# gyhandy/Neural-Sim-NeRF

Hardware: AMD Instinct MI355X
Metric: Mray-samples/sec at 400x400, 64+128 samples, 8x256 MLP (higher is better)
Workload: dtype f16x2

## Files before the change

### neural_sim_nerf_amd/csrc/nsr_kernels.hip

```cpp
#include <hip/hip_runtime.h>
#include <stdint.h>
#include "nsr_device.h"

#if !defined(NSR_UNIT_F32) && !defined(NSR_UNIT_H2) && !defined(NSR_UNIT_B3) && !defined(NSR_UNIT_X16)
#define NSR_UNIT_F32 1
#define NSR_UNIT_H2 1
#define NSR_UNIT_B3 1
#define NSR_UNIT_X16 1
#endif
#ifndef NSR_UNIT_F32
#define NSR_UNIT_F32 0
#endif
#ifndef NSR_UNIT_H2
#define NSR_UNIT_H2 0
#endif
#ifndef NSR_UNIT_B3
#define NSR_UNIT_B3 0
#endif
#ifndef NSR_UNIT_X16
#define NSR_UNIT_X16 0
#endif
#define NSR_CAT_(a, b) a##b
#define NSR_CAT(a, b) NSR_CAT_(a, b)

// ... 87 lines not shown
  const char* p = rg.smem + rg.cslot * kSlabBytes + lane * 16;
#pragma unroll
  for (int c = 0; c < 4; ++c) A0[c] = *(const f32x4*)(p + c * 1024);
}

template <int U>
__device__ __forceinline__ void ring_load_quarter(const Ring& rg, f32x4 (&A)[4], int lane) {
  const char* p = rg.smem + rg.cslot * kSlabBytes + U * kStepBytes + lane * 16;
#pragma unroll
  for (int c = 0; c < 4; ++c) A[c] = *(const f32x4*)(p + c * 1024);
}

template <int NS = kRingSlots>
__device__ __forceinline__ void ring_advance(Ring& rg, f32x4 (&A)[4], int lane) {
  asm volatile("s_waitcnt vmcnt(%0) lgkmcnt(0)" ::"n"(4 * (NS - 2)) : "memory");
#ifndef NSR_EXP_NOBARRIER
  __builtin_amdgcn_s_barrier();
#endif
  rg.cslot = (rg.cslot + 1 == NS) ? 0 : rg.cslot + 1;
  const char* p = rg.smem + rg.cslot * kSlabBytes + lane * 16;
#pragma unroll
  for (int c = 0; c < 4; ++c) A[c] = *(const f32x4*)(p + c * 1024);
}

#define NSR_MFMA(a, b, c) __builtin_amdgcn_mfma_f32_32x32x2f32((a), (b), (c), 0, 0, 0)
__device__ __forceinline__ f32x16 mfma_op(float a, float b, f32x16 c) { return __builtin_amdgcn_mfma_f32_32x32x2f32(a, b, c, 0, 0, 0); }
__device__ __forceinline__ f32x4 mfma_op(float a, float b, f32x4 c) { return __builtin_amdgcn_mfma_f32_16x16x4f32(a, b, c, 0, 0, 0); }

template <int NMO, int KK0, int KK1, bool ZERO = false, int NACC, typename BOp, typename AccT>
__device__ __forceinline__ void consume(const f32x4 (&A)[4], int step, BOp bop, AccT (&acc)[NACC]) {
#pragma unroll
  for (int kk = KK0; kk < KK1; ++kk)
#pragma unroll
    for (int c = 0; c < 4; ++c) {
      const int n = 4 * step + c, tq = n / NMO, mo = n % NMO;
      if (ZERO && tq == 0 && kk == 0) acc[mo] = mfma_op(A[c][kk], bop(4 * tq + kk), AccT{0});
      else acc[mo] = mfma_op(A[c][kk], bop(4 * tq + kk), acc[mo]);
    }
}

#define NSR_PIN() __builtin_amdgcn_sched_barrier(0)
#define NSR_SGB(mask, n) __builtin_amdgcn_sched_group_barrier((mask), (n), 0)
#define NSR_MASK_VALU 0x002
#define NSR_MASK_SALU 0x004
#define NSR_MASK_MFMA 0x008
#define NSR_MASK_VMEM 0x010
#define NSR_MASK_DSRD 0x100
template <int N_MFMA>
__device__ __forceinline__ void step_pattern() {
#pragma unroll
  for (int i = 0; i < N_MFMA; ++i) {
    NSR_SGB(NSR_MASK_MFMA, 1);
    NSR_SGB(NSR_MASK_DSRD, 1);
    NSR_SGB(NSR_MASK_VALU, 2);
  }
}
template <int N_MFMA>
__device__ __forceinline__ void step_pattern_dma() {
#pragma unroll
  for (int i = 0; i < N_MFMA; ++i) {
    NSR_SGB(NSR_MASK_MFMA, 1);
    NSR_SGB(NSR_MASK_DSRD, 1);
    NSR_SGB(NSR_MASK_VMEM, 1);
    NSR_SGB(NSR_MASK_SALU, 3);
    NSR_SGB(NSR_MASK_VALU, 2);
  }
}

template <int NMO, int NTQ, int NS = kRingSlots, bool ZERO = false, int NACC, typename BOp, typename AccT>
__device__ __forceinline__ void seg(Ring& rg, f32x4 (&A0)[4], f32x4 (&A1)[4], BOp bop, AccT (&acc)[NACC],
                                    int lane) {
  static_assert((NMO * NTQ) % 16 == 0, "a segment is a whole number of slabs");
#pragma unroll
  for (int s = 0; s < NMO * NTQ / 4; s += 4) {
    NSR_PIN(); ring_load_quarter<1>(rg, A1, lane); consume<NMO, 0, 4, ZERO>(A0, s, bop, acc);     step_pattern<16>();
    NSR_PIN(); ring_load_quarter<2>(rg, A0, lane); consume<NMO, 0, 4, ZERO>(A1, s + 1, bop, acc); step_pattern<16>();
    NSR_PIN(); ring_load_quarter<3>(rg, A1, lane); consume<NMO, 0, 4, ZERO>(A0, s + 2, bop, acc); step_pattern<16>();
    NSR_PIN(); consume<NMO, 0, 1, ZERO>(A1, s + 3, bop, acc);
    NSR_PIN(); ring_advance<NS>(rg, A0, lane);
    ring_issue<NS>(rg); consume<NMO, 1, 4, ZERO>(A1, s + 3, bop, acc); step_pattern_dma<12>();
    NSR_PIN();
  }
}

template <int NG>
struct BRegs16 {
  const f32x16 (&v)[NG];
  __device__ __forceinline__ float operator()(int t) const { return v[t >> 4][t & 15]; }
};
template <int N>
struct BArr {
  const float (&v)[N];
  __device__ __forceinline__ float operator()(int t) const { return v[t]; }
};
struct BViews {
  const f32x16 (&v)[8];
  const float (&ed)[16];
  __device__ __forceinline__ float operator()(int t) const { return t < 128 ? v[(t & 127) >> 4][t & 15] : ed[t & 15]; }
};

__device__ __forceinline__ int aux_half(int lane) { return opaque_v((lane >> 5) * 4); }

template <int NMO>
__device__ __forceinline__ void load_bias(const float* bias, int h4 , f32x16 (&acc)[NMO]) {
#pragma unroll
  for (int mo = 0; mo < NMO; ++mo)
#pragma unroll
    for (int rq = 0; rq < 4; ++rq) {
      f32x4 v = *(const f32x4*)(bias + (mo * 4 + rq) * 8 + h4);
      acc[mo][rq * 4 + 0] = v[0];
      acc[mo][rq * 4 + 1] = v[1];
      acc[mo][rq * 4 + 2] = v[2];
      acc[mo][rq * 4 + 3] = v[3];
    }
}

#include "nsr_b3.inc"
#include "nsr_h2.inc"

constexpr int kMlpF32 = 0;
constexpr int kMlpB3 = 1;
constexpr int kMlpH2 = 2;

template <int NMO>
__device__ __forceinline__ uint4 relu_mask(const f32x16 (&acc)[NMO]) {
  unsigned w[4] = {0u, 0u, 0u, 0u};
#pragma unroll
  for (int mo = 0; mo < NMO; ++mo)
#pragma unroll
    for (int r = 0; r < 16; ++r) {
      const int on = max(__float_as_int(acc[mo][r]), 0) - 1;
      w[mo >> 1] = __builtin_amdgcn_alignbit(w[mo >> 1], (unsigned)on, 31);
    }
  return make_uint4(w[0], w[1], w[2], w[3]);
}

__device__ __forceinline__ float enc_trig(float a, int k) {
  const double kMagic = 6755399441055744.0;
  const double t = (double)a * 0.63661977236758134308;
  const double tm = t + kMagic;
  const int n = __double2loint(tm) + k;
  const double f = t - (tm - kMagic);
  const float r = (float)(f * 1.57079632679489661923);
  const float z = r * r;
  float ps = __builtin_fmaf(-1.9515295891e-4f, z, 8.3321608736e-3f);
  ps = __builtin_fmaf(ps, z, -1.6666654611e-1f);
  ps = __builtin_fmaf(ps * z, r, r);
  float pc = __builtin_fmaf(2.443315711809948e-5f, z, -1.388731625493765e-3f);
  pc = __builtin_fmaf(pc, z, 4.166664568298827e-2f);
  pc = __builtin_fmaf(pc * z, z, __builtin_fmaf(-0.5f, z, 1.0f));
  const float v = (n & 1) ? pc : ps;
  return __uint_as_float(__float_as_uint(v) ^ ((unsigned)(n & 2) << 30));
}

__device__ __forceinline__ float enc_domain(float x, int nfreq) {
  return __builtin_fabsf(x) < ldexpf(1.0f, 25 - nfreq) ? x : __builtin_nanf("");
}

__device__ __forceinline__ float enc_poison(float px, float py, float pz, float vx, float vy, float vz) {
  const float a = (enc_domain(px, kMultires) * 0.0f + enc_domain(py, kMultires) * 0.0f) + enc_domain(pz, kMultires) * 0.0f;
  const float b = (enc_domain(vx, kMultiresViews) * 0.0f + enc_domain(vy, kMultiresViews) * 0.0f) +
                  enc_domain(vz, kMultiresViews) * 0.0f;
  return __builtin_fabsf(a + b);
}

template <bool CAPTURE, int MODE = kMlpF32>
__device__ __forceinline__ void mlp_pass(Ring& rg, const float* aux, f32x4 (&A0)[4], f32x4 (&A1)[4], int lane,
                                         float px, float py, float pz, float vx, float vy, float vz,
                                         float (&raw)[4], uint4* mask_dst = nullptr , int mask_tid = 0,
                                         long long* tp = nullptr ) {
#ifdef NSR_PHASE_TIMING
  long long tpl = clock64();
#define NSR_TP(i) do { if (tp) { const long long t_ = clock64(); tp[i] += t_ - tpl; tpl = t_; } } while (0)
#else
#define NSR_TP(i) do { } while (0)
#endif
  const int h = lane >> 5;
  const int h4 = aux_half(lane);
  const float poison = enc_poison(px, py, pz, vx, vy, vz);
  float e[32];
  float ed[16];
  {
    const float p[3] = {px, py, pz};
    const float v[3] = {vx, vy, vz};
#pragma unroll
    for (int L = 0; L < kMultires; ++L)
#pragma unroll
      for (int ax = 0; ax < 3; ++ax) e[3 * L + ax] = enc_trig(enc_domain(p[ax], kMultires) * (float)(1 << L), h);
#pragma unroll
    for (int L = 0; L < kMultiresViews; ++L)
#pragma unroll
      for (int ax = 0; ax < 3; ++ax) ed[3 * L + ax] = enc_trig(enc_domain(v[ax], kMultiresViews) * (float)(1 << L), h);
    e[30] = h ? pz : px;
    e[31] = h ? 0.0f : py;
    ed[12] = h ? vz : vx;
    ed[13] = h ? 0.0f : vy;
    ed[14] = 0.0f;
    ed[15] = 0.0f;
  }

  f32x16 acc[8];
  f32x16 in[8];
  auto enc_src = [&](int kb, int i) { return e[(8 * kb + i) & 31]; };
  auto in_src = [&](int kb, int i) { return in[(kb >> 1) & 7][8 * (kb & 1) + i]; };
  constexpr bool B3 = MODE == kMlpB3;
  constexpr bool H2M = MODE == kMlpH2;
  float amax = 0.0f;
  const float* h2s = aux + kAuxH2Scale;
#if NSR_H2_SCHED == 3 && !defined(NSR_EXP_H2_NOFRAG) && !defined(NSR_EXP_H2_HALFBARRIER) && !defined(NSR_EXP_H2_NOSPLIT)
  constexpr bool TAIL = H2M && !CAPTURE;
#else
  constexpr bool TAIL = false;
#endif
  static_assert(kAuxBiasV == kAuxBias + 9 * 256, "the views layer's bias follows feature_linear's: 'bias of layer L + 1' for L = 8");
  NSR_TP(0);
  load_bias<8>(aux + kAuxBias, h4, acc);
  NSR_TP(2);
  if constexpr (B3) gemm_b3<8, 2>(rg, A0, A1, enc_src, acc, lane);
  else if constexpr (TAIL)
    gemm_h2_tail<4>(rg, A0, A1, enc_src, H2Scale{{h2s[0], 0.0f}, 4}, acc, lane, amax, H2Tail{acc, in, 0, h2_lds_base(aux + kAuxBias + 256, h4)});
  else if constexpr (H2M) gemm_h2<8, 4>(rg, A0, A1, enc_src, H2Scale{{h2s[0], 0.0f}, 4}, acc, lane, amax);
  else seg<8, 8>(rg, A0, A1, BArr<32>{e}, acc, lane);
  NSR_TP(1);
  if (CAPTURE) mask_dst[mask_tid] = relu_mask<8>(acc);
  if constexpr (!TAIL) {
#pragma unroll
    for (int mo = 0; mo < 8; ++mo) in[mo] = relu16(acc[mo]);
  }

  float alpha_part = 0.0f;
#pragma unroll 1
  for (int L = 1; L <= 8; ++L) {
    if constexpr (!TAIL) load_bias<8>(aux + kAuxBias + L * 256, h4, acc);
    NSR_TP(2);
    if (L == 5) {
      if constexpr (B3) gemm_b3<8, 2>(rg, A0, A1, enc_src, acc, lane);
      else if constexpr (H2M) gemm_h2<8, 4>(rg, A0, A1, enc_src, H2Scale{{h2s[9], 0.0f}, 4}, acc, lane, amax);
      else seg<8, 8>(rg, A0, A1, BArr<32>{e}, acc, lane);
      NSR_TP(1);
    }
    if (L == 8) {
      const float* wa = aux + kAuxWAlpha;
#pragma unroll
      for (int tq = 0; tq < 32; ++tq) {
        f32x4 w = *(const f32x4*)(wa + tq * 8 + h4);
#pragma unroll
        for (int kk = 0; kk < 4; ++kk)
          alpha_part = __builtin_fmaf(w[kk], in[(4 * tq + kk) >> 4][(4 * tq + kk) & 15], alpha_part);
      }
    }
    if constexpr (B3) gemm_b3<8, 8>(rg, A0, A1, in_src, acc, lane);
    else if constexpr (TAIL)
      gemm_h2_tail<16>(rg, A0, A1, in_src, H2Scale{{h2s[L], 0.0f}, 16}, acc, lane, amax,
                       H2Tail{acc, in, (L == 8) ? (int)0x80000000 : 0, h2_lds_base(aux + kAuxBias + (L + 1) * 256, h4)});
    else if constexpr (H2M) gemm_h2<8, 16>(rg, A0, A1, in_src, H2Scale{{h2s[L], 0.0f}, 16}, acc, lane, amax);
    else seg<8, 32>(rg, A0, A1, BRegs16<8>{in}, acc, lane);
    NSR_TP(1);
    if (CAPTURE && L < 8) mask_dst[L * 256 + mask_tid] = relu_mask<8>(acc);
    if constexpr (!TAIL) {
      const int thr = (L == 8) ? (int)0x80000000 : 0;
#pragma unroll
      for (int mo = 0; mo < 8; ++mo) in[mo] = clamp_bits16(acc[mo], thr);
    }
  }

  f32x16 av[4];
  if constexpr (TAIL) {
#pragma unroll
    for (int mo = 0; mo < 4; ++mo) av[mo] = acc[mo];
  } else {
    load_bias<4>(aux + kAuxBiasV, h4, av);
  }
  NSR_TP(2);
  if constexpr (B3) {
    auto v_src = [&](int kb, int i) {
      return kb < 16 ? in[(kb >> 1) & 7][8 * (kb & 1) + i] : (kb < 18 ? ed[(8 * (kb - 16) + i) & 15] : 0.0f);
    };
    gemm_b3<4, 5>(rg, A0, A1, v_src, av, lane);
  } else if constexpr (H2M) {
    auto v_src = [&](int kb, int i) { return kb < 16 ? in[(kb >> 1) & 7][8 * (kb & 1) + i] : ed[(8 * (kb - 16) + i) & 15]; };
    gemm_h2<4, 18>(rg, A0, A1, v_src, H2Scale{{h2s[10], h2s[11]}, 16}, av, lane, amax);
  } else {
    seg<4, 36>(rg, A0, A1, BViews{in, ed}, av, lane);
  }
  NSR_TP(1);
  if (CAPTURE) mask_dst[8 * 256 + mask_tid] = relu_mask<4>(av);

  float part[4] = {0.0f, 0.0f, 0.0f, alpha_part};
  if constexpr (H2M) {
    const float ov = amax > kH2Max ? __builtin_nanf("") : 0.0f;
    part[0] = part[1] = part[2] = ov;
    part[3] = alpha_part + ov;
  }
#pragma unroll
  for (int c = 0; c < 3; ++c) {
    const float* wr = aux + kAuxWRgb + c * 128;
#pragma unroll
    for (int mo = 0; mo < 4; ++mo)
#pragma unroll
      for (int rq = 0; rq < 4; ++rq) {
        f32x4 w = *(const f32x4*)(wr + (mo * 4 + rq) * 8 + h4);
#pragma unroll
        for (int ri = 0; ri < 4; ++ri)
          part[c] = __builtin_fmaf(w[ri], fmaxf(av[mo][rq * 4 + ri], 0.0f), part[c]);
      }
  }
#pragma unroll
  for (int c = 0; c < 4; ++c) {
    float other = __shfl_xor(part[c], 32);
    float lo_half = h ? other : part[c];
    float hi_half = h ? part[c] : other;
    raw[c] = ((lo_half + hi_half) + aux[(c < 3) ? (kAuxBRgb + c) : kAuxBAlpha]) + poison;
  }
  NSR_TP(3);
#undef NSR_TP
}

template <int NSS, int NFS>
struct ItemStateT {
  static constexpr int kNS = NSS, kNF = NFS;
  float tcoarse[NSS];
  float ufine[128];
  float ray[2][16];
  float zc[2][NSS];
  float rawc[2][NSS][4];
  float w0[2][NSS];
  float cdf[2][NSS];
  float zs[2][128];
  float zf[2][NFS];
  float rawf[2][NFS][4];
  float alpha[2][NFS];
  float wf[2][NFS];
  float tf[2][NFS];
  float om[2][NFS];
  float bwd_scratch[2][NFS][2];
  float psum[2][NFS / 32][12];
  float gnorm[2];
  float res[2][8];
};
typedef ItemStateT<64, 192> ItemState;
typedef ItemStateT<128, 256> ItemStateBig;
static_assert(sizeof(ItemState) == 23048, "the YCB-V layout is part of the shipped kernels' LDS budget");
template <int NS> struct ItemStateFor { typedef ItemState type; };
template <> struct ItemStateFor<128> { typedef ItemStateBig type; };

__device__ __forceinline__ float sigmoidf_(float x) { return 1.0f / (1.0f + expf(-x)); }

template <int S, int R = 2, int STRIDE = S, typename ST>
__device__ __forceinline__ void composite(ST& st, const float* z, float* raw, float* wout, float* tout, int tid,
                                          const float* noise = nullptr ,
                                          long long row0 = 0, int valid = R) {
  static_assert(S % 8 == 0, "scan is unrolled by 8");
  for (int idx = tid; idx < R * S; idx += 256) {
    const int r = idx / S, i = idx - r * S;
    const float* zr = z + r * STRIDE;
    float dist = (i < S - 1) ? (zr[i + 1] - zr[i]) : 1e10f;
    dist = dist * st.ray[r][11];
    float* q = raw + (r * STRIDE + i) * 4;
    if (noise) q[3] = q[3] + noise[(row0 + (r < valid ? r : 0)) * S + i];
    const float sigma = fmaxf(q[3], 0.0f);
    const float a = 1.0f - expf(-sigma * dist);
    st.alpha[r][i] = a;
    st.om[r][i] = (1.0f - a) + 1e-10f;
    q[0] = sigmoidf_(q[0]);
    q[1] = sigmoidf_(q[1]);
    q[2] = sigmoidf_(q[2]);
  }
  __syncthreads();
  if ((tid & 63) == 0 && tid < 64 * R) {
    const int r = tid >> 6;
    double T = 1.0;
#pragma unroll 1
    for (int i0 = 0; i0 < S; i0 += 8) {
      double f[8];
#pragma unroll
      for (int k = 0; k < 8; ++k) f[k] = (double)st.om[r][i0 + k];
#pragma unroll
      for (int k = 0; k < 8; ++k) {
        tout[r * STRIDE + i0 + k] = (float)T;
        T = T * f[k];
      }
    }
  }
  __syncthreads();
  if (tid < 64 * R) {
    const int r = tid >> 6, l = tid & 63;
    const float* zr = z + r * STRIDE;
    const float* q = raw + r * STRIDE * 4;
    float cr = 0.f, cg = 0.f, cb = 0.f, depth = 0.f, acc = 0.f;
#pragma unroll
    for (int i = l; i < S; i += 64) {
      const float w = st.alpha[r][i] * tout[r * STRIDE + i];
      wout[r * STRIDE + i] = w;
      cr = cr + w * q[i * 4 + 0];
      cg = cg + w * q[i * 4 + 1];
      cb = cb + w * q[i * 4 + 2];
      depth = depth + w * zr[i];
      acc = acc + w;
    }
#pragma unroll
    for (int m = 32; m >= 1; m >>= 1) {
      cr += __shfl_xor(cr, m); cg += __shfl_xor(cg, m); cb += __shfl_xor(cb, m);
      depth += __shfl_xor(depth, m); acc += __shfl_xor(acc, m);
    }
    if (l == 0) {
      const float qd = depth / acc;
      float disp;
      if (qd != qd) disp = qd;
      else disp = 1.0f / fmaxf(1e-10f, qd);
      if (st.ray[r][12] != 0.0f) {
        const float bg = 1.0f - acc;
        cr = cr + bg; cg = cg + bg; cb = cb + bg;
      }
      st.res[r][0] = cr; st.res[r][1] = cg; st.res[r][2] = cb;
      st.res[r][3] = disp; st.res[r][4] = acc; st.res[r][5] = depth;
    }
  }
  __syncthreads();
}

template <int R, int NI, int NS, typename ST, typename BinsFn>
__device__ __forceinline__ void sample_pdf_item_ns(ST& st, const float* ufine, const float* w, int wstride, BinsFn bins,
                                                   int64_t* inds_out, int64_t inds_stride, int tid, int valid_rays,
                                                   const float* u_rays, long long row0, int write_mask) {
// ... 251 lines not shown
    __syncthreads();
    if (tid < 2 * NS) st.zc[r][i] = zn;
    __syncthreads();
  }
}

__device__ __forceinline__ void gen_ray(const float* __restrict__ c2w, float fx, float fy, float cx, float cy,
                                        int row, int col, float (&o)[3], float (&d)[3]) {
  const float dx = ((float)col - cx) / fx;
  const float dy = -(((float)row - cy) / fy);
  const float dz = -1.0f;
#pragma unroll
  for (int a = 0; a < 3; ++a) {
    d[a] = ((dx * c2w[a * 4 + 0]) + (dy * c2w[a * 4 + 1])) + (dz * c2w[a * 4 + 2]);
    o[a] = c2w[a * 4 + 3];
  }
}

struct RenderArgs {
  const float* nets;
  long long net_stride;
  const float* aux[2];
  const float* tcoarse;
  const float* ufine;
  const float* rays_o;
  const float* rays_d;
  const float* c2w;
  float fx, fy, cx, cy;
  int H, W;
  long long n_rays;
  float near_, far_;
  int fine;
  int camera;
  int white_bkgd;
  int lindisp;
  float *rgb, *disp, *acc, *rgb0, *disp0, *acc0, *z_std;
  float *dbg_w0, *dbg_zs, *dbg_zf, *dbg_raw0, *dbg_raw;
  long long* dbg_inds;
  float* zf_scratch;
  int chunk;
  unsigned* sched_flags;
  unsigned* status;
  int super_lg;
  int spin_max;
  unsigned epoch;
  unsigned* epoch_counter;
  unsigned long long* work_counter;
  const float* viewdirs;
  const float* t_rand;
  const float* u_rays;
  const float* noise0;
  const float* noise1;
  const float* near_rays;
  const float* far_rays;
  unsigned long long* ovf_items;
  unsigned* ovf_stat;
  unsigned ovf_cap;
  const unsigned long long* item_list;
  const unsigned* item_count;
  unsigned item_cap;
};

__device__ __forceinline__ void load_aux(char* smem, const RenderArgs& a, int tid) {
  float* dst = (float*)(smem + kLdsAux);
  for (int i = tid; i < kAuxFloats; i += 256) {
    dst[i] = a.aux[0][i];
    dst[kAuxFloats + i] = a.aux[1][i];
  }
}

#if NSR_UNIT_F32
__global__ void k_set_args(const RenderArgs a, RenderArgs* dst) {
  *dst = a;
  *a.work_counter = 0ull;
  if (a.ovf_stat) a.ovf_stat[0] = 0u;
  if (a.epoch_counter) dst->epoch = *a.epoch_counter = *a.epoch_counter % 4094u + 1u;
}
#endif

constexpr long long kItemMask = (1ll << 62) - 1;
__device__ __forceinline__ long long queue_next_item(const RenderArgs& q) {
  const unsigned long long v = atomicAdd(q.work_counter, 1ull);
  if (q.item_list) {
    unsigned n = *q.item_count;
    n = n < q.item_cap ? n : q.item_cap;
    return v < (unsigned long long)n ? (long long)q.item_list[v] : -1ll;
  }
  return v < (unsigned long long)((q.n_rays + 1) >> 1) ? (long long)(v | (3ull << 62)) : -1ll;
}
__device__ __forceinline__ long long queue_item_of(const RenderArgs& q, unsigned long long v) {
  if (q.item_list) {
    unsigned n = *q.item_count;
    n = n < q.item_cap ? n : q.item_cap;
    return v < (unsigned long long)n ? (long long)q.item_list[v] : -1ll;
  }
  return v < (unsigned long long)((q.n_rays + 1) >> 1) ? (long long)(v | (3ull << 62)) : -1ll;
}
__device__ __forceinline__ long long queue_items(const RenderArgs& q) {
  if (q.item_list) { const unsigned n = *q.item_count; return (long long)(n < q.item_cap ? n : q.item_cap); }
  return (q.n_rays + 1) >> 1;
}
__device__ __forceinline__ void range_mark(int* ovf, float chk, int lane) {
#ifndef NSR_EXP_NO_RANGE
  if (chk != chk && lane < 32) atomicAdd(ovf, 1);
#endif
}
__device__ __forceinline__ unsigned range_report(const RenderArgs& a, int* ovf, long long item, int valid) {
#ifdef NSR_EXP_NO_RANGE
  return 0u;
#endif
  const int p0 = ovf[0], p1 = valid == 2 ? ovf[1] : 0;
  if ((p0 | p1) != 0 && a.ovf_stat) {
    const unsigned long long mask = (p0 ? 1ull : 0ull) | (p1 ? 2ull : 0ull);
    const unsigned n = atomicAdd(a.ovf_stat, 1u);
    atomicAdd(a.ovf_stat + 1, (unsigned)(p0 + p1));
    if (n < a.ovf_cap) {
      a.ovf_items[n] = (unsigned long long)item | (mask << 62);
      atomicAdd(a.ovf_stat + 2, (unsigned)((p0 != 0) + (p1 != 0)));
    } else {
      atomicAdd(a.ovf_stat + 3, 1u);
      return (unsigned)mask;
    }
  }
  return 0u;
}
__device__ __forceinline__ void range_poison(const RenderArgs& a, long long ray0, unsigned mask) {
  const float qn = __builtin_nanf("");
  for (int r = 0; r < 2; ++r) {
    if (!((mask >> r) & 1u)) continue;
    const long long rr = ray0 + r;
    float* const v3[2] = {a.rgb, a.rgb0};
    float* const v1[5] = {a.disp, a.acc, a.disp0, a.acc0, a.z_std};
    for (int k = 0; k < 2; ++k) if (v3[k]) { v3[k][rr * 3] = qn; v3[k][rr * 3 + 1] = qn; v3[k][rr * 3 + 2] = qn; }
    for (int k = 0; k < 5; ++k) if (v1[k]) v1[k][rr] = qn;
  }
}

__device__ __forceinline__ void wave_lds_sync() {
  __builtin_amdgcn_fence(__ATOMIC_RELEASE, "wavefront");
  __builtin_amdgcn_wave_barrier();
  __builtin_amdgcn_fence(__ATOMIC_ACQUIRE, "wavefront");
}
__device__ __forceinline__ void lds_barrier() { asm volatile("s_waitcnt lgkmcnt(0)\n\ts_barrier" ::: "memory"); }

template <typename ST>
struct FwdItemExtra {
  float om[2][ST::kNS];
  float tf[2][ST::kNS];
  float zf[2][ST::kNF];
  float ray[2][16];
  float res[2][8];
  long long pend;
  long long next;
};

template <int S>
__device__ __forceinline__ void composite_wave(const float* ry, const float* zr, float* q, float* wr, float* tr, float* omr,
                                               int lane, const float* noise ,
                                               float (&res)[6]) {
  static_assert(S % 8 == 0, "scan is unrolled by 8");
  constexpr int K = (S + 63) / 64;
  float al[K];
#pragma unroll
  for (int k = 0; k < K; ++k) {
    const int i = lane + 64 * k;
    al[k] = 0.0f;
    if (i < S) {
      float dist = (i < S - 1) ? (zr[i + 1] - zr[i]) : 1e10f;
      dist = dist * ry[11];
      if (noise) q[i * 4 + 3] = q[i * 4 + 3] + noise[i];
      const float sigma = fmaxf(q[i * 4 + 3], 0.0f);
      const float a = 1.0f - expf(-sigma * dist);
      al[k] = a;
      omr[i] = (1.0f - a) + 1e-10f;
      q[i * 4 + 0] = sigmoidf_(q[i * 4 + 0]);
      q[i * 4 + 1] = sigmoidf_(q[i * 4 + 1]);
      q[i * 4 + 2] = sigmoidf_(q[i * 4 + 2]);
    }
  }
  wave_lds_sync();
  if (lane == 0) {
    double T = 1.0;
#pragma unroll 1
    for (int i0 = 0; i0 < S; i0 += 8) {
      double f[8];
#pragma unroll
      for (int k = 0; k < 8; ++k) f[k] = (double)omr[i0 + k];
#pragma unroll
      for (int k = 0; k < 8; ++k) {
        tr[i0 + k] = (float)T;
        T = T * f[k];
      }
    }
  }
  wave_lds_sync();
  float cr = 0.f, cg = 0.f, cb = 0.f, depth = 0.f, acc = 0.f;
#pragma unroll
  for (int k = 0; k < K; ++k) {
    const int i = lane + 64 * k;
    if (i < S) {
      const float w = al[k] * tr[i];
      wr[i] = w;
      cr = cr + w * q[i * 4 + 0];
      cg = cg + w * q[i * 4 + 1];
      cb = cb + w * q[i * 4 + 2];
      depth = depth + w * zr[i];
      acc = acc + w;
    }
  }
#pragma unroll
  for (int m = 32; m >= 1; m >>= 1) {
    cr += __shfl_xor(cr, m); cg += __shfl_xor(cg, m); cb += __shfl_xor(cb, m);
    depth += __shfl_xor(depth, m); acc += __shfl_xor(acc, m);
  }
  const float qd = depth / acc;
  float disp;
  if (qd != qd) disp = qd;
  else disp = 1.0f / fmaxf(1e-10f, qd);
  if (ry[12] != 0.0f) {
    const float bg = 1.0f - acc;
    cr = cr + bg; cg = cg + bg; cb = cb + bg;
  }
  res[0] = cr; res[1] = cg; res[2] = cb; res[3] = disp; res[4] = acc; res[5] = depth;
  wave_lds_sync();
}

template <int NI, int NS>
__device__ __forceinline__ void sample_pdf_wave(const float* w, const float* zc, float* x, float* pdf, float* cdf, float* zs,
                                                const float* u ,
                                                int64_t* inds_out , int lane) {
  constexpr int NW = NS - 2, NC = NS - 1;
  constexpr int NVEC = NW / 8, SILP = NVEC / 4;
  constexpr int KW = (NW + 63) / 64;
  float xv[KW];
#pragma unroll
  for (int k = 0; k < KW; ++k) {
    const int i = lane + 64 * k;
    xv[k] = 0.0f;
    if (i < NW) { xv[k] = w[i] + 1e-5f; x[i] = xv[k]; }
  }
  wave_lds_sync();
  const int j = lane & 7;
  float lj;
  if constexpr (NS == 64) {
    const float p0 = ((x[j] + x[32 + j]) + x[40 + j]) + x[48 + j];
    lj = ((p0 + x[8 + j]) + x[16 + j]) + x[24 + j];
  } else {
    float ps[4] = {0.0f, 0.0f, 0.0f, 0.0f};
#pragma unroll
    for (int i = 0; i < SILP; ++i)
#pragma unroll
      for (int k = 0; k < 4; ++k) ps[k] = ps[k] + x[(i * 4 + k) * 8 + j];
#pragma unroll
    for (int v = SILP * 4; v < NVEC; ++v) ps[0] = ps[0] + x[v * 8 + j];
    lj = ((ps[0] + ps[1]) + ps[2]) + ps[3];
  }
  float total = 0.0f;
#pragma unroll
  for (int i = NVEC * 8; i < NW; ++i) total = total + x[i];
#pragma unroll
  for (int jj = 0; jj < 8; ++jj) total = total + __shfl(lj, jj);
#pragma unroll
  for (int k = 0; k < KW; ++k) {
    const int i = lane + 64 * k;
    if (i < NW) pdf[i] = xv[k] / total;
  }
  wave_lds_sync();
  if (lane == 0) {
    double run = 0.0;
    cdf[0] = 0.0f;
#pragma unroll 1
    for (int i0 = 0; i0 < NVEC * 8; i0 += 8) {
      double f[8];
#pragma unroll
      for (int k = 0; k < 8; ++k) f[k] = (double)pdf[i0 + k];
#pragma unroll
      for (int k = 0; k < 8; ++k) { run = run + f[k]; cdf[i0 + k + 1] = (float)run; }
    }
#pragma unroll
    for (int i = NVEC * 8; i < NW; ++i) { run = run + (double)pdf[i]; cdf[i + 1] = (float)run; }
  }
  wave_lds_sync();
#pragma unroll
  for (int kk = 0; kk < (NI + 63) / 64; ++kk) {
    const int k = lane + 64 * kk;
    if (k < NI) {
      const float uu = u[k];
      int lo = 0, hi = NC;
      while (lo < hi) {
        const int mid = (lo + hi) >> 1;
        if (cdf[NSR_IDX(mid, NC)] <= uu) lo = mid + 1; else hi = mid;
      }
      const int ind = lo;
      const int below = NSR_IDX(max(ind - 1, 0), NC);
      const int above = NSR_IDX(min(ind, NC - 1), NC);
      const float c0 = cdf[below], c1 = cdf[above];
      const float b0 = 0.5f * (zc[below + 1] + zc[below]), b1 = 0.5f * (zc[above + 1] + zc[above]);
      float denom = c1 - c0;
      if (denom < 1e-5f) denom = 1.0f;
      const float t = (uu - c0) / denom;
      zs[NSR_IDX(k, 128)] = b0 + t * (b1 - b0);
      if (inds_out) inds_out[k] = (int64_t)ind;
    }
  }
  wave_lds_sync();
}

template <int NI, int NS>
__device__ __forceinline__ void merge_wave(const float* zc, const float* zs, float* zf, int lane) {
  constexpr int NF = NS + NI;
  constexpr bool kPow2 = (NI & (NI - 1)) == 0 && (NS & (NS - 1)) == 0;
  constexpr int K = (NF + 63) / 64;
  int bad = 0;
#pragma unroll
  for (int kk = 0; kk < K; ++kk) {
    const int k = lane + 64 * kk;
    if (k < NS - 1) bad |= !(zc[k] <= zc[k + 1]);
    else if (k >= NS && k < NF - 1) bad |= !(zs[k - NS] <= zs[k - NS + 1]);
  }
  const bool any_bad = __builtin_amdgcn_ballot_w64(bad != 0) != 0;
  if (!any_bad) {
#pragma unroll
    for (int kk = 0; kk < K; ++kk) {
      const int k = lane + 64 * kk;
      if (k < NS) {
        const float x = zc[k];
        int lb = 0;
        if constexpr (kPow2) {
#pragma unroll
          for (int sft = NI / 2; sft > 0; sft >>= 1) lb += (zs[lb + sft - 1] < x) ? sft : 0;
          lb += (zs[lb] < x) ? 1 : 0;
        } else {
          int hi = NI;
          while (lb < hi) { const int mid = (lb + hi) >> 1; if (zs[NSR_IDX(mid, NI)] < x) lb = mid + 1; else hi = mid; }
        }
        zf[NSR_IDX(k + lb, NF)] = x;
      } else if (k < NF) {
        const float x = zs[k - NS];
        int ub = 0;
        if constexpr (kPow2) {
#pragma unroll
          for (int sft = NS / 2; sft > 0; sft >>= 1) ub += (zc[ub + sft - 1] <= x) ? sft : 0;
          ub += (zc[ub] <= x) ? 1 : 0;
        } else {
          int hi = NS;
          while (ub < hi) { const int mid = (ub + hi) >> 1; if (zc[NSR_IDX(mid, NS)] <= x) ub = mid + 1; else hi = mid; }
        }
        zf[NSR_IDX((k - NS) + ub, NF)] = x;
      }
    }
  } else {
#pragma unroll 1
    for (int kk = 0; kk < K; ++kk) {
      const int k = lane + 64 * kk;
      if (k < NF) {
        const float x = (k < NS) ? zc[k] : zs[k - NS];
        int rank = 0;
        for (int jx = 0; jx < NS; ++jx) {
          const float y = zc[jx];
          rank += (y < x) || (y == x && jx < k);
        }
        for (int jx = 0; jx < NI; ++jx) {
          const float y = zs[jx];
          rank += (y < x) || (y == x && (jx + NS) < k);
        }
        zf[NSR_IDX(rank, NF)] = x;
      }
    }
  }
  wave_lds_sync();
}

#ifdef NSR_PHASE_TIMING
#define NSR_T(i) do { if (threadIdx.x == 0) { const long long t_ = clock64(); tacc[i] += t_ - tlast; tlast = t_; } } while (0)
#else
#define NSR_T(i) do { } while (0)
#endif

template <int MODE, int NI = 128, int NS = 64>
__device__ __forceinline__ void render32_body(const RenderArgs* __restrict__ ap, char* smem) {
  constexpr bool B3 = MODE == kMlpB3;
  constexpr int NF = NS + NI;
  constexpr int NP = (2 * NF + 127) / 128;
  constexpr int NPC = (2 * NS + 127) / 128;
  constexpr int LNS = NS == 32 ? 5 : (NS == 64 ? 6 : 7);
  typedef typename ItemStateFor<NS>::type ST;
  static_assert((NS == 32 || NS == 64 || NS == 128) && NF % 32 == 0 && NS <= ST::kNS && NF <= ST::kNF,
                "a wave's points belong to one ray; the item state holds kNS coarse / kNF fine samples per ray");
  const RenderArgs& a_setup = *ap;
#ifdef NSR_PHASE_TIMING
  long long tacc[8] = {0, 0, 0, 0, 0, 0, 0, 0};
  long long tpass[4] = {0, 0, 0, 0};
  long long tlast = clock64();
#define NSR_TPASS tpass
#else
#define NSR_TPASS nullptr
#endif
  const int tid0 = threadIdx.x;
  const int lane = tid0 & 63;
  const int wave = __builtin_amdgcn_readfirstlane(tid0 >> 6);
  const int j = lane & 31;
  ST& st = *(ST*)(smem + kLdsState);

  const long long n_rays = a_setup.n_rays;
  if ((long long)blockIdx.x >= queue_items(a_setup)) return;
  const int fine = a_setup.fine;
  typedef FwdItemExtra<ST> XT;
  static_assert(offsetof(ST, res) - offsetof(ST, bwd_scratch) >= sizeof(XT) && offsetof(ST, bwd_scratch) % 8 == 0 &&
                offsetof(XT, pend) % 8 == 0, "the forward scratch lives in the item state's backward scratch");
  XT& xs = *(XT*)&st.bwd_scratch[0][0][0];

  Ring rg;
  ring_init(rg, smem, a_setup.nets, a_setup.net_stride, fine ? NPC + NP : NPC, wave, lane);
  rg.pn0 = NPC; rg.pn1 = NPC + NP;

  f32x4 A0[4], A1[4];
  if constexpr (B3) ring_start<kRingSlots, kStreamSlabsB3, kStreamSlabsB3Bwd>(rg, A0, lane);
  else if constexpr (MODE == kMlpH2) ring_start<kRingSlots, kStreamSlabs, kStreamSlabs, kH2RingLag>(rg, A0, lane);
  else ring_start(rg, A0, lane);

  load_aux(smem, a_setup, tid0);
  if (tid0 < NS) st.tcoarse[tid0] = a_setup.tcoarse[tid0];
  if (tid0 < NI) st.ufine[tid0] = a_setup.ufine[tid0];
  if (tid0 == 0) xs.pend = -1ll;
  __syncthreads();
  const float* aux_c = (const float*)(smem + kLdsAux);

  long long* item_slot = (long long*)&st.ray[0][14];
  auto next_item = [&]() -> long long {
    if (opaque_v(tid0) == 0) *item_slot = queue_next_item(*opaque_s(ap));
    lds_barrier();
    const long long v = uniform64(*item_slot);
    lds_barrier();
    return v;
  };

  auto fine_wave = [&](long long pk, int pp, int r) {
    const RenderArgs& a = *opaque_s(ap);
    const long long ray0 = (pk & kItemMask) * 2;
    const int valid = (ray0 + 1 < n_rays) ? 2 : 1;
    const int wmask = (int)((unsigned long long)pk >> 62) & (valid == 2 ? 3 : 1);
    const float* ry = pp ? xs.ray[r] : st.ray[r];
    const float* zr = pp ? xs.zf[r] : st.zf[r];
    float* q = &st.rawf[r][0][0];
    if (a.dbg_raw && ((wmask >> r) & 1)) {
      for (int idx = lane; idx < NF * 4; idx += 64) a.dbg_raw[(ray0 + r) * (NF * 4) + idx] = q[idx];
      wave_lds_sync();
    }
    float res[6];
    composite_wave<NF>(ry, zr, q, st.wf[r], st.tf[r], st.om[r], lane,
                       a.noise1 ? a.noise1 + (ray0 + (r < valid ? r : 0)) * NF : nullptr, res);
    if (lane == 0) {
#pragma unroll
      for (int c = 0; c < 6; ++c) st.res[r][c] = res[c];
    }
  };
  auto fine_out = [&](long long pk, int pp) {
    const RenderArgs& a = *opaque_s(ap);
    const int tid = opaque_v(tid0);
    const long long item = pk & kItemMask;
    const long long ray0 = item * 2;
    const int valid = (ray0 + 1 < n_rays) ? 2 : 1;
    const int wmask = (int)((unsigned long long)pk >> 62) & (valid == 2 ? 3 : 1);
    if (tid < 16 && ((wmask >> (tid >> 3)) & 1)) {
      const int r = tid >> 3, c = tid & 7;
      const long long rr = ray0 + r;
      const float v = st.res[r][c];
      if (c < 3) { if (a.rgb) a.rgb[rr * 3 + c] = v; }
      else if (c == 3) { if (a.disp) a.disp[rr] = v; }
      else if (c == 4) { if (a.acc) a.acc[rr] = v; }
    }
    if (MODE == kMlpH2 && tid == 0) {
      int* povf = (int*)(pp ? &xs.ray[1][14] : &st.ray[1][14]);
      if (const unsigned m = range_report(a, povf, item, valid)) range_poison(a, ray0, m);
    }
  };

  long long packed = next_item();
  int pass = 0;
  int par = 0;
#pragma unroll 1
  while (packed != -1ll) {
    const long long item = packed & kItemMask;
    const long long ray0 = item * 2;
    const int valid = (ray0 + 1 < n_rays) ? 2 : 1;
    const int wmask = (int)((unsigned long long)packed >> 62) & (valid == 2 ? 3 : 1);
    auto wr = [&](int r) { return ((wmask >> r) & 1) != 0; };
    float (*const ray)[16] = par ? xs.ray : st.ray;
    float* const zf = par ? &xs.zf[0][0] : &st.zf[0][0];
    int* const ovf = (int*)&ray[1][14];
    if (pass == 0) {
      const RenderArgs& a = *opaque_s(ap);
      const int tid = opaque_v(tid0);
      const float near_ = a.near_, far_ = a.far_;
      if (tid < 2) {
        const long long rr = ray0 + (tid < valid ? tid : 0);
        float o[3], d[3];
        if (a.camera) {
          const long long hw = (long long)a.H * a.W;
          const long long v = rr / hw;
          const int pix = (int)(rr - v * hw);
          gen_ray(a.c2w + v * 12, a.fx, a.fy, a.cx, a.cy, pix / a.W, pix % a.W, o, d);
        } else {
#pragma unroll
          for (int c = 0; c < 3; ++c) { o[c] = a.rays_o[rr * 3 + c]; d[c] = a.rays_d[rr * 3 + c]; }
        }
        const float nrm = sqrtf(((d[0] * d[0]) + (d[1] * d[1])) + (d[2] * d[2]));
        const float* vd = a.camera ? nullptr : a.viewdirs;
#pragma unroll
        for (int c = 0; c < 3; ++c) {
          ray[tid][c] = o[c]; ray[tid][3 + c] = d[c];
          ray[tid][6 + c] = vd ? vd[rr * 3 + c] : d[c] / nrm;
        }
        ray[tid][9] = a.near_rays ? a.near_rays[rr] : near_;
        ray[tid][10] = a.near_rays ? a.far_rays[rr] : far_;
        ray[tid][11] = nrm;
        ray[tid][12] = a.white_bkgd ? 1.0f : 0.0f;
      }
      if (MODE == kMlpH2 && (tid == 64 || tid == 65)) ovf[tid - 64] = 0;
      if (tid < 2 * NS) {
        const int r = tid >> LNS, i = tid & (NS - 1);
        const float t = st.tcoarse[i];
        const long long rb = ray0 + (r < valid ? r : 0);
        st.zc[r][i] = coarse_z(a.near_rays ? a.near_rays[rb] : near_, a.near_rays ? a.far_rays[rb] : far_, t, a.lindisp);
      }
      lds_barrier();
      if (a.t_rand) perturb_coarse_z<NS>(st, a.t_rand, ray0, valid, tid);
      NSR_T(0);
    }

    {
      int r, i;
      const float* zsrc;
      float* dst;
      bool real = true;
      if ((NPC == 1) ? (pass == 0) : (pass < NPC)) {
        if constexpr (NS == 64) {
          r = wave >> 1; i = 32 * (wave & 1) + j;
        } else {
          int q0 = 128 * pass + 32 * wave;
          if (2 * NS % 128 != 0 && q0 >= 2 * NS) { q0 = 2 * NS - 32; real = false; }
          r = q0 >> LNS; i = (q0 & (NS - 1)) + j;
        }
        zsrc = &st.zc[r][i]; dst = st.rawc[r][i];
      } else {
        int q0 = 128 * (pass - NPC) + 32 * wave;
        if (2 * NF % 128 != 0 && q0 >= 2 * NF) { q0 = 2 * NF - 32; real = false; }
        r = q0 / NF; i = q0 - r * NF + j;
        zsrc = &zf[r * ST::kNF + i]; dst = st.rawf[r][i];
      }
      const float z = *zsrc;
      const float* ry = ray[r];
      float raw[4];
      mlp_pass<false, MODE>(rg, aux_c + (((NPC == 1) ? (pass == 0) : (pass < NPC)) ? 0 : kAuxFloats), A0, A1, lane, ry[0] + ry[3] * z, ry[1] + ry[4] * z,
               ry[2] + ry[5] * z, ry[6], ry[7], ry[8], raw, nullptr, 0, NSR_TPASS);
      if (lane < 32 && real) *(f32x4*)dst = f32x4{raw[0], raw[1], raw[2], raw[3]};
      if constexpr (MODE == kMlpH2) { if (real) range_mark(ovf + r, (raw[0] + raw[1]) + (raw[2] + raw[3]), lane); }
    }
    NSR_T(1);

    const RenderArgs& a = *opaque_s(ap);
    const int tid = opaque_v(tid0);
    if (NPC > 1 && pass < NPC - 1) {
      ++pass;
    } else if ((NPC == 1) ? (pass == 0) : (pass < NPC)) {
      lds_barrier();
      const long long pend = fine ? uniform64(xs.pend) : -1ll;
      const bool puller = fine && tid == 192;
      unsigned long long ticket = 0ull;
      if (puller) ticket = atomicAdd(a.work_counter, 1ull);
      if (wave < 2) {
        const int r = wave;
        float* q = &st.rawc[r][0][0];
        if (a.dbg_raw0 && wr(r)) {
          for (int idx = lane; idx < NS * 4; idx += 64) a.dbg_raw0[(ray0 + r) * (NS * 4) + idx] = q[idx];
          wave_lds_sync();
        }
        float res[6];
        composite_wave<NS>(ray[r], st.zc[r], q, st.w0[r], xs.tf[r], xs.om[r], lane,
                           a.noise0 ? a.noise0 + (ray0 + (r < valid ? r : 0)) * NS : nullptr, res);
        if (lane == 0) {
#pragma unroll
          for (int c = 0; c < 6; ++c) xs.res[r][c] = res[c];
        }
        if (a.dbg_w0 && wr(r))
          for (int idx = lane; idx < NS; idx += 64) a.dbg_w0[(ray0 + r) * NS + idx] = st.w0[r][idx];
        NSR_T(2);
        if (fine) {
#ifdef NSR_PHASE_TIMING
          int64_t* inds = nullptr;
#else
          int64_t* inds = (int64_t*)a.dbg_inds;
#endif
          sample_pdf_wave<NI, NS>(&st.w0[r][1], st.zc[r], xs.tf[r], xs.om[r], st.cdf[r], st.zs[r],
                                  a.u_rays ? a.u_rays + (ray0 + (r < valid ? r : 0)) * 128 : st.ufine,
                                  (inds && wr(r)) ? inds + (ray0 + r) * NI : nullptr, lane);
          NSR_T(3);
          const float sd = zstd_wave<NI>(st, r, lane);
          if (lane == 0 && wr(r) && a.z_std) a.z_std[ray0 + r] = sd;
          if (a.dbg_zs && wr(r))
            for (int k = lane; k < NI; k += 64) a.dbg_zs[(ray0 + r) * NI + k] = st.zs[r][k];
          NSR_T(4);
          merge_wave<NI, NS>(st.zc[r], st.zs[r], zf + r * ST::kNF, lane);
          if (a.dbg_zf && wr(r))
            for (int k = lane; k < NF; k += 64) a.dbg_zf[(ray0 + r) * NF + k] = zf[r * ST::kNF + k];
          NSR_T(5);
        }
      } else if (pend != -1ll) {
#ifdef NSR_PHASE_TIMING
        const long long t0_ = clock64();
#endif
        fine_wave(pend, par ^ 1, wave - 2);
#ifdef NSR_PHASE_TIMING
        if (threadIdx.x == 128) tacc[7] += clock64() - t0_;
#endif
      }
      if (puller) xs.next = queue_item_of(a, ticket);
      lds_barrier();
      if (pend != -1ll) fine_out(pend, par ^ 1);
      if (tid < 16 && wr(tid >> 3)) {
        const int r = tid >> 3, c = tid & 7;
        const long long rr = ray0 + r;
        const float v = xs.res[r][c];
        float* rgb_dst = fine ? a.rgb0 : a.rgb;
        float* disp_dst = fine ? a.disp0 : a.disp;
        float* acc_dst = fine ? a.acc0 : a.acc;
        if (c < 3) { if (rgb_dst) rgb_dst[rr * 3 + c] = v; }
        else if (c == 3) { if (disp_dst) disp_dst[rr] = v; }
        else if (c == 4) { if (acc_dst) acc_dst[rr] = v; }
      }
      NSR_T(6);
      if (!fine) {
        if (MODE == kMlpH2 && tid == 0) { if (const unsigned m = range_report(a, ovf, item, valid)) range_poison(a, ray0, m); }
        if constexpr (NPC > 1) pass = 0;
        packed = next_item(); continue;
      }
      pass = NPC;
    } else if (pass < NPC + NP - 1) {
      ++pass;
    } else {
      if (tid == 0) xs.pend = packed;
      pass = 0;
      par ^= 1;
      packed = uniform64(xs.next);
    }
  }
  if (fine) {
    lds_barrier();
    const long long pend = uniform64(xs.pend);
    if (pend != -1ll) {
      if (wave < 2) fine_wave(pend, par ^ 1, wave);
      lds_barrier();
      fine_out(pend, par ^ 1);
    }
    NSR_T(6);
  }
  asm volatile("s_waitcnt vmcnt(0)" ::: "memory");
#ifdef NSR_PHASE_TIMING
  if (tid0 == 128 && a_setup.dbg_raw == nullptr && a_setup.dbg_inds) a_setup.dbg_inds[blockIdx.x * 8 + 7] = tacc[7];
  if (tid0 == 0 && a_setup.dbg_raw == nullptr && a_setup.dbg_inds)
    for (int i = 0; i < 7; ++i) a_setup.dbg_inds[blockIdx.x * 8 + i] = tacc[i];
  if (tid0 == 0 && a_setup.dbg_raw == nullptr && a_setup.dbg_inds)
    for (int i = 0; i < 4; ++i) a_setup.dbg_inds[(long long)gridDim.x * 8 + blockIdx.x * 4 + i] = tpass[i];
#endif
#undef NSR_TPASS
}

#define NSR_RENDER_KERNEL_1(NAME, ...)                                                               \
  __global__ void __launch_bounds__(256, 1) NAME(const RenderArgs* __restrict__ ap) {                \
    extern __shared__ __attribute__((aligned(16))) char smem[];                                      \
    render32_body<__VA_ARGS__>(ap, smem);                                                            \
  }
#define NSR_RENDER_KERNEL_0(NAME, ...) __global__ void __launch_bounds__(256, 1) NAME(const RenderArgs* __restrict__ ap);
#define NSR_RENDER_KERNEL(UNIT, NAME, ...) NSR_CAT(NSR_RENDER_KERNEL_, UNIT)(NAME, __VA_ARGS__)
NSR_RENDER_KERNEL(NSR_UNIT_F32, k_render, kMlpF32)
NSR_RENDER_KERNEL(NSR_UNIT_B3, k_render_b3, kMlpB3)
NSR_RENDER_KERNEL(NSR_UNIT_H2, k_render_h2, kMlpH2)
NSR_RENDER_KERNEL(NSR_UNIT_H2, k_render_h2_n64, kMlpH2, 64)
NSR_RENDER_KERNEL(NSR_UNIT_H2, k_render_h2_n32, kMlpH2, 32)
NSR_RENDER_KERNEL(NSR_UNIT_B3, k_render_b3_n64, kMlpB3, 64)
NSR_RENDER_KERNEL(NSR_UNIT_B3, k_render_b3_n32, kMlpB3, 32)
NSR_RENDER_KERNEL(NSR_UNIT_H2, k_render_h2_n96, kMlpH2, 96, 64)
NSR_RENDER_KERNEL(NSR_UNIT_B3, k_render_b3_n96, kMlpB3, 96, 64)
NSR_RENDER_KERNEL(NSR_UNIT_H2, k_render_h2_c32_n64, kMlpH2, 64, 32)
NSR_RENDER_KERNEL(NSR_UNIT_B3, k_render_b3_c32_n64, kMlpB3, 64, 32)
NSR_RENDER_KERNEL(NSR_UNIT_H2, k_render_h2_c128_n128, kMlpH2, 128, 128)
NSR_RENDER_KERNEL(NSR_UNIT_B3, k_render_b3_c128_n128, kMlpB3, 128, 128)
#undef NSR_RENDER_KERNEL
#undef NSR_RENDER_KERNEL_0
#undef NSR_RENDER_KERNEL_1

__device__ __forceinline__ f32x16 apply_mask(f32x16 x, unsigned word, int shift) {
  f32x16 r;
#pragma unroll
  for (int i = 0; i < 16; ++i)
    r[i] = ((word >> (31 - (shift + i))) & 1u) ? 0.0f : x[i];
  return r;
}

template <int NFREQ>
__device__ __forceinline__ void embed_bwd(const float (&x)[3], const float* G , int h,
                                          float (&out)[3]) {
  out[0] = h ? 0.0f : G[3 * NFREQ];
  out[1] = h ? 0.0f : G[3 * NFREQ + 1];
  out[2] = h ? G[3 * NFREQ] : 0.0f;
#pragma unroll
  for (int L = 0; L < NFREQ; ++L)
#pragma unroll
// ... 1797 lines not shown
```

Baseline: 290.6.

## Pair sin/cos positional encoding and precompute per-ray direction encoding in LDS

In the H2 tail path, the point encoding now computes sine and cosine from one range reduction and polynomial evaluation. The two half-waves then exchange values with permlane32_swap, so each lane evaluates half as many trig reductions. The view-direction encoding is constant per ray, so it is computed once per ray by a few threads into LDS scratch and loaded as four b128 reads per lane instead of being recomputed for every sample. This removes redundant transcendental work at the cost of an extra LDS region, cross-lane swaps and an added LDS dependency before the views layer.

```diff
diff --git a/neural_sim_nerf_amd/csrc/nsr_kernels.hip b/neural_sim_nerf_amd/csrc/nsr_kernels.hip
--- a/neural_sim_nerf_amd/csrc/nsr_kernels.hip
+++ b/neural_sim_nerf_amd/csrc/nsr_kernels.hip
@@ -263,6 +263,24 @@
   const float v = (n & 1) ? pc : ps;
   return __uint_as_float(__float_as_uint(v) ^ ((unsigned)(n & 2) << 30));
 }
+__device__ __forceinline__ void enc_trig_pair(float a, float& s, float& c) {
+  const double kMagic = 6755399441055744.0;
+  const double t = (double)a * 0.63661977236758134308;
+  const double tm = t + kMagic;
+  const int n = __double2loint(tm), n1 = n + 1;
+  const double f = t - (tm - kMagic);
+  const float r = (float)(f * 1.57079632679489661923);
+  const float z = r * r;
+  float ps = __builtin_fmaf(-1.9515295891e-4f, z, 8.3321608736e-3f);
+  ps = __builtin_fmaf(ps, z, -1.6666654611e-1f);
+  ps = __builtin_fmaf(ps * z, r, r);
+  float pc = __builtin_fmaf(2.443315711809948e-5f, z, -1.388731625493765e-3f);
+  pc = __builtin_fmaf(pc, z, 4.166664568298827e-2f);
+  pc = __builtin_fmaf(pc * z, z, __builtin_fmaf(-0.5f, z, 1.0f));
+  const float v = (n & 1) ? pc : ps, v1 = (n1 & 1) ? pc : ps;
+  s = __uint_as_float(__float_as_uint(v) ^ ((unsigned)(n & 2) << 30));
+  c = __uint_as_float(__float_as_uint(v1) ^ ((unsigned)(n1 & 2) << 30));
+}
 
 __device__ __forceinline__ float enc_domain(float x, int nfreq) {
   return __builtin_fabsf(x) < ldexpf(1.0f, 25 - nfreq) ? x : __builtin_nanf("");
@@ -275,16 +293,56 @@
   return __builtin_fabsf(a + b);
 }
 
+__device__ __forceinline__ void enc_points_paired(const float (&p)[3], int h, float (&e)[32]) {
+  static_assert(kMultires % 2 == 0, "levels come in pairs");
+#pragma unroll
+  for (int q = 0; q < kMultires / 2; ++q) {
+    const float f = h ? (float)(2 << (2 * q)) : (float)(1 << (2 * q));
+#pragma unroll
+    for (int ax = 0; ax < 3; ++ax) {
+      float s, c;
+      enc_trig_pair(enc_domain(p[ax], kMultires) * f, s, c);
+      const auto x = __builtin_amdgcn_permlane32_swap(__float_as_uint(s), __float_as_uint(c), false, false);
+      e[3 * (2 * q) + ax] = __uint_as_float(x[0]);
+      e[3 * (2 * q + 1) + ax] = __uint_as_float(x[1]);
+    }
+  }
+}
+
+__device__ __forceinline__ float enc_dir_slot(const float* v , int h, int i) {
+  static_assert(3 * kMultiresViews == 12, "slots 12..15 of ed[] are the raw direction and padding");
+  if (i < 3 * kMultiresViews) return enc_trig(enc_domain(v[i % 3], kMultiresViews) * (float)(1 << (i / 3)), h);
+  return i == 12 ? (h ? v[2] : v[0]) : ((i == 13 && !h) ? v[1] : 0.0f);
+}
+
 template <bool CAPTURE, int MODE = kMlpF32>
 __device__ __forceinline__ void mlp_pass(Ring& rg, const float* aux, f32x4 (&A0)[4], f32x4 (&A1)[4], int lane,
                                          float px, float py, float pz, float vx, float vy, float vz,
                                          float (&raw)[4], uint4* mask_dst = nullptr , int mask_tid = 0,
-                                         long long* tp = nullptr ) {
+                                         long long* tp = nullptr ,
+                                         const float* dirs = nullptr ) {
 #ifdef NSR_PHASE_TIMING
   long long tpl = clock64();
 #define NSR_TP(i) do { if (tp) { const long long t_ = clock64(); tp[i] += t_ - tpl; tpl = t_; } } while (0)
 #else
 #define NSR_TP(i) do { } while (0)
+#endif
+  constexpr bool B3 = MODE == kMlpB3;
+  constexpr bool H2M = MODE == kMlpH2;
+#if NSR_H2_SCHED == 3 && !defined(NSR_EXP_H2_NOFRAG) && !defined(NSR_EXP_H2_HALFBARRIER) && !defined(NSR_EXP_H2_NOSPLIT)
+  constexpr bool TAIL = H2M && !CAPTURE;
+#else
+  constexpr bool TAIL = false;
+#endif
+#ifdef NSR_EXP_ENC_NOPAIR
+  constexpr bool PAIRED = false;
+#else
+  constexpr bool PAIRED = TAIL;
+#endif
+#ifdef NSR_EXP_ENC_NODIRS
+  constexpr bool DIRS = false;
+#else
+  constexpr bool DIRS = TAIL;
 #endif
   const int h = lane >> 5;
   const int h4 = aux_half(lane);
@@ -294,35 +352,44 @@
   {
     const float p[3] = {px, py, pz};
     const float v[3] = {vx, vy, vz};
-#pragma unroll
-    for (int L = 0; L < kMultires; ++L)
-#pragma unroll
-      for (int ax = 0; ax < 3; ++ax) e[3 * L + ax] = enc_trig(enc_domain(p[ax], kMultires) * (float)(1 << L), h);
-#pragma unroll
-    for (int L = 0; L < kMultiresViews; ++L)
-#pragma unroll
-      for (int ax = 0; ax < 3; ++ax) ed[3 * L + ax] = enc_trig(enc_domain(v[ax], kMultiresViews) * (float)(1 << L), h);
+    if constexpr (PAIRED) {
+      enc_points_paired(p, h, e);
+    } else {
+#pragma unroll
+      for (int L = 0; L < kMultires; ++L)
+#pragma unroll
+        for (int ax = 0; ax < 3; ++ax) e[3 * L + ax] = enc_trig(enc_domain(p[ax], kMultires) * (float)(1 << L), h);
+    }
+    if constexpr (!DIRS) {
+#pragma unroll
+      for (int L = 0; L < kMultiresViews; ++L)
+#pragma unroll
+        for (int ax = 0; ax < 3; ++ax) ed[3 * L + ax] = enc_trig(enc_domain(v[ax], kMultiresViews) * (float)(1 << L), h);
+    }
     e[30] = h ? pz : px;
     e[31] = h ? 0.0f : py;
-    ed[12] = h ? vz : vx;
-    ed[13] = h ? 0.0f : vy;
-    ed[14] = 0.0f;
-    ed[15] = 0.0f;
-  }
+    if constexpr (!DIRS) {
+      ed[12] = h ? vz : vx;
+      ed[13] = h ? 0.0f : vy;
+      ed[14] = 0.0f;
+      ed[15] = 0.0f;
+    }
+  }
+#ifdef NSR_PHASE_TIMING
+#pragma unroll
+  for (int t = 0; t < 32; ++t) asm volatile("" ::"v"(e[t]));
+  if constexpr (!DIRS) {
+#pragma unroll
+    for (int t = 0; t < 16; ++t) asm volatile("" ::"v"(ed[t]));
+  }
+#endif
 
   f32x16 acc[8];
   f32x16 in[8];
   auto enc_src = [&](int kb, int i) { return e[(8 * kb + i) & 31]; };
   auto in_src = [&](int kb, int i) { return in[(kb >> 1) & 7][8 * (kb & 1) + i]; };
-  constexpr bool B3 = MODE == kMlpB3;
-  constexpr bool H2M = MODE == kMlpH2;
   float amax = 0.0f;
   const float* h2s = aux + kAuxH2Scale;
-#if NSR_H2_SCHED == 3 && !defined(NSR_EXP_H2_NOFRAG) && !defined(NSR_EXP_H2_HALFBARRIER) && !defined(NSR_EXP_H2_NOSPLIT)
-  constexpr bool TAIL = H2M && !CAPTURE;
-#else
-  constexpr bool TAIL = false;
-#endif
   static_assert(kAuxBiasV == kAuxBias + 9 * 256, "the views layer's bias follows feature_linear's: 'bias of layer L + 1' for L = 8");
   NSR_TP(0);
   load_bias<8>(aux + kAuxBias, h4, acc);
@@ -381,6 +448,14 @@
     for (int mo = 0; mo < 4; ++mo) av[mo] = acc[mo];
   } else {
     load_bias<4>(aux + kAuxBiasV, h4, av);
+  }
+  if constexpr (DIRS) {
+#pragma unroll
+    for (int t = 0; t < 4; ++t) {
+      const f32x4 d = *(const f32x4*)(dirs + 16 * h + 4 * t);
+#pragma unroll
+      for (int i = 0; i < 4; ++i) ed[4 * t + i] = d[i];
+    }
   }
   NSR_TP(2);
   if constexpr (B3) {
@@ -938,6 +1013,7 @@
   float res[2][8];
   long long pend;
   long long next;
+  float dirs[2][2][2][16];
 };
 
 template <int S>
@@ -1193,7 +1269,8 @@
   const int fine = a_setup.fine;
   typedef FwdItemExtra<ST> XT;
   static_assert(offsetof(ST, res) - offsetof(ST, bwd_scratch) >= sizeof(XT) && offsetof(ST, bwd_scratch) % 8 == 0 &&
-                offsetof(XT, pend) % 8 == 0, "the forward scratch lives in the item state's backward scratch");
+                offsetof(XT, pend) % 8 == 0 && (kLdsState + offsetof(ST, bwd_scratch) + offsetof(XT, dirs)) % 16 == 0,
+                "the forward scratch lives in the item state's backward scratch; a direction block is read as four b128");
   XT& xs = *(XT*)&st.bwd_scratch[0][0][0];
 
   Ring rg;
@@ -1311,6 +1388,9 @@
         st.zc[r][i] = coarse_z(a.near_rays ? a.near_rays[rb] : near_, a.near_rays ? a.far_rays[rb] : far_, t, a.lindisp);
       }
       lds_barrier();
+      if constexpr (MODE == kMlpH2) {
+        if (tid >= 64 && tid < 128) xs.dirs[par][(tid >> 5) & 1][(tid >> 4) & 1][tid & 15] = enc_dir_slot(&ray[(tid >> 5) & 1][6], (tid >> 4) & 1, tid & 15);
+      }
       if (a.t_rand) perturb_coarse_z<NS>(st, a.t_rand, ray0, valid, tid);
       NSR_T(0);
     }
@@ -1339,7 +1419,7 @@
       const float* ry = ray[r];
       float raw[4];
       mlp_pass<false, MODE>(rg, aux_c + (((NPC == 1) ? (pass == 0) : (pass < NPC)) ? 0 : kAuxFloats), A0, A1, lane, ry[0] + ry[3] * z, ry[1] + ry[4] * z,
-               ry[2] + ry[5] * z, ry[6], ry[7], ry[8], raw, nullptr, 0, NSR_TPASS);
+               ry[2] + ry[5] * z, ry[6], ry[7], ry[8], raw, nullptr, 0, NSR_TPASS, &xs.dirs[par][r][0][0]);
       if (lane < 32 && real) *(f32x4*)dst = f32x4{raw[0], raw[1], raw[2], raw[3]};
       if constexpr (MODE == kMlpH2) { if (real) range_mark(ovf + r, (raw[0] + raw[1]) + (raw[2] + raw[3]), lane); }
     }
```

Result: no change. 292.7, median of 6 (+0.8%).
